# sd196821/QuadSim

Measured on AMD Instinct MI355X. Metric: env-steps/sec at N parallel envs (1/2/4/8 GPU); per-step state L2 err vs NumPy ref, higher is better.
Workload: dtype f32

## Files before the change

### quadsim_amd/csrc/step_kernels.hpp

```cpp
#pragma once

namespace {

#ifndef QS_BLOCK
#define QS_BLOCK 256
#endif
constexpr int kBlock = QS_BLOCK;
#ifndef QS_PREP_MAX_TILES
#define QS_PREP_MAX_TILES 1365
#endif
constexpr int64_t kPrepMaxTiles = QS_PREP_MAX_TILES;
#ifndef QS_SPLIT_MAX_ENVS
#define QS_SPLIT_MAX_ENVS 131072
#endif
constexpr int64_t kSplitMaxEnvs = QS_SPLIT_MAX_ENVS;

struct StepArgs {
    float *st;
    float *par;
    const float *actions;
    float *obs;
    float *reward;
    uint8_t *done;
    uint8_t *flags;
    float *term_obs;
    float *term_state;
    float *slab;
    int64_t n;
    int64_t tile0, tile_end;
    int64_t dbg_shift;
    int64_t io_env0, io_n;
    int64_t T;
    uint64_t step_idx;
    unsigned long long *ctr;
    uint64_t gid0;
    EnvConst C;
    RandCfg rc;
    Par par_nom;
    int auto_reset;
    int randomise;
    float nominal_obs[12];
    const float *init;
    unsigned *owner;
    unsigned *err;
    unsigned long long *stamps;
    unsigned long long stamp_cap, stamp_tiles;
};

__device__ __forceinline__ void load_env(const float *__restrict__ st, int64_t tile, int lane, Env &e)
{
    const float *b = st + tile * (int64_t)(kRecWords * kTile) + lane;
#pragma unroll
    for (int i = 0; i < 13; ++i) e.sc[i] = b[(F_SC + i) * kTile];
#pragma unroll
    for (int i = 0; i < 13; ++i) e.st[i] = b[(F_ST + i) * kTile];
#pragma unroll
    for (int i = 0; i < 4; ++i) e.uc[i] = b[(F_UC + i) * kTile];
#pragma unroll
    for (int i = 0; i < 4; ++i) e.ut[i] = b[(F_UT + i) * kTile];
#pragma unroll
    for (int i = 0; i < 4; ++i) e.qd[i] = b[(F_QD + i) * kTile];
    e.ls = b[F_LS * kTile];
    e.t = b[F_T * kTile];
}

__device__ __forceinline__ void load_env_or_nominal(const StepArgs &A, int64_t tile, int lane, bool active, Env &e)
{
    if (active) load_env(A.st, tile, lane, e);
    else { nominal_init(e.sc, e.st); for (int i = 0; i < 4; ++i) { e.uc[i] = 0.0f; e.ut[i] = 0.0f; e.qd[i] = i == 0; } e.ls = 0.0f; e.t = 0.0f; }
}

__device__ __forceinline__ void store_env(float *__restrict__ st, int64_t tile, int lane, const Env &e)
{
    float *b = st + tile * (int64_t)(kRecWords * kTile) + lane;
#pragma unroll
    for (int i = 0; i < 13; ++i) QS_ST(&b[(F_SC + i) * kTile], e.sc[i]);
#pragma unroll
    for (int i = 0; i < 13; ++i) QS_ST(&b[(F_ST + i) * kTile], e.st[i]);
#pragma unroll
    for (int i = 0; i < 4; ++i) QS_ST(&b[(F_UC + i) * kTile], e.uc[i]);
#pragma unroll
    for (int i = 0; i < 4; ++i) QS_ST(&b[(F_UT + i) * kTile], e.ut[i]);
#pragma unroll
    for (int i = 0; i < 4; ++i) QS_ST(&b[(F_QD + i) * kTile], e.qd[i]);
    QS_ST(&b[F_LS * kTile], e.ls);
    QS_ST(&b[F_T * kTile], e.t);
}

__device__ __forceinline__ Par load_par(const float *__restrict__ par, int64_t tile, int lane)
{
    const float *b = par + tile * (int64_t)(kParWords * kTile) + lane;
    Par P;
    P.m = b[0]; P.Ixx = b[kTile]; P.Iyy = b[2 * kTile]; P.Izz = b[3 * kTile];
    return P;
}

__device__ __forceinline__ void store_par(float *__restrict__ par, int64_t tile, int lane, const Par &P)
{
    float *b = par + tile * (int64_t)(kParWords * kTile) + lane;
    b[0] = P.m; b[kTile] = P.Ixx; b[2 * kTile] = P.Iyy; b[3 * kTile] = P.Izz;
}

struct TileLane { int lane; int64_t tile, env; bool active; };
__device__ __forceinline__ TileLane tile_lane(int64_t n)
{
    const int lane = threadIdx.x & (kTile - 1);
    const int64_t tile = (int64_t)blockIdx.x * (kBlock / kTile) + (threadIdx.x >> 6);
    const int64_t env = tile * kTile + lane;
    return {lane, tile, env, env < n};
}

__device__ __forceinline__ void store_obs(float *__restrict__ obs, int64_t env, const float o[12])
{
    typedef float f4 __attribute__((ext_vector_type(4)));
    f4 *p = reinterpret_cast<f4 *>(obs + env * 12);
    QS_SO(&p[0], (f4{o[0], o[1], o[2], o[3]}));
    QS_SO(&p[1], (f4{o[4], o[5], o[6], o[7]}));
    QS_SO(&p[2], (f4{o[8], o[9], o[10], o[11]}));
}

__device__ __forceinline__ void store_obs_cached(float *__restrict__ obs, int64_t env, const float o[12])
{
    float4 *p = reinterpret_cast<float4 *>(obs + env * 12);
    p[0] = make_float4(o[0], o[1], o[2], o[3]);
    p[1] = make_float4(o[4], o[5], o[6], o[7]);
    p[2] = make_float4(o[8], o[9], o[10], o[11]);
}

__device__ __forceinline__ uint64_t step_counter_begin(const StepArgs &A, int64_t tile) { return A.ctr[tile]; }
__device__ __forceinline__ uint64_t step_counter_begin_vmem(const StepArgs &A, int64_t tile)
{
    int zero;
    asm("v_mov_b32 %0, 0" : "=v"(zero));
    return A.ctr[tile + zero];
}
__device__ __forceinline__ void step_counter_end(const StepArgs &A, int64_t tile, int lane, uint64_t k)
{
    if (lane == 0) A.ctr[tile] = k + (uint64_t)A.T;
}

constexpr unsigned kUnowned = 0xffffffffu;
__device__ __forceinline__ unsigned chain_owner_request(const StepArgs &A, int64_t tile)
{
    const unsigned *p = A.owner ? A.owner + tile : reinterpret_cast<const unsigned *>(A.ctr + tile);
    const unsigned v = __hip_atomic_load(p, __ATOMIC_RELAXED, __HIP_MEMORY_SCOPE_AGENT);
    return A.owner ? v : kUnowned;
}

__device__ __forceinline__ bool chain_owner_mismatch(const StepArgs &A, int64_t tile, int lane, unsigned own)
{
    const unsigned xcc = __builtin_amdgcn_s_getreg((3 << 11) | (0 << 6) | 20) & 15u;
    if (own == kUnowned) {
        unsigned seen = kUnowned;
        if (lane == 0) {
            unsigned expect = kUnowned;
            __hip_atomic_compare_exchange_strong(&A.owner[tile], &expect, xcc, __ATOMIC_RELAXED, __ATOMIC_RELAXED, __HIP_MEMORY_SCOPE_AGENT);
            seen = expect;
        }
        own = __builtin_amdgcn_readfirstlane(seen);
        if (own == kUnowned) return false;
    }
    if (own != xcc) {
        if (lane == 0) __hip_atomic_fetch_or(A.err, 1u, __ATOMIC_RELAXED, __HIP_MEMORY_SCOPE_SYSTEM);
        return true;
    }
    return false;
}

__device__ __forceinline__ bool chain_tile_misplaced(const StepArgs &A, int64_t tile, int lane)
{
    if (!A.owner) return false;
    return chain_owner_mismatch(A, tile, lane, chain_owner_request(A, tile));
}

__device__ __forceinline__ int64_t launch_tile(const StepArgs &A, int64_t b)
{
    const int64_t nt = A.tile_end - A.tile0;
    b += A.dbg_shift;
    b -= (b >= nt) ? nt : 0;
    return A.tile0 + b;
}

template <bool PARAMS, int RMODE>
__device__ __forceinline__ void maybe_reset(Env &e, Par &P, const StepArgs &A, int64_t env, uint64_t k, float obs[12], unsigned flags,
                                            bool &done, bool write_term);

template <int INTEG, bool PARAMS, int RMODE>
__device__ __forceinline__ void step_and_maybe_reset(Env &e, Par &P, const float a[4], const StepArgs &A, int64_t env,
                                                     uint64_t k, float obs[12], float &reward, unsigned &flags,
                                                     bool &done, bool write_term)
{
    env_step<INTEG>(e, a, P, A.C, obs, reward, flags);
    maybe_reset<PARAMS, RMODE>(e, P, A, env, k, obs, flags, done, write_term);
}

template <bool PARAMS, int RMODE>
__device__ __forceinline__ void maybe_reset(Env &e, Par &P, const StepArgs &A, int64_t env, uint64_t k, float obs[12], unsigned flags,
                                            bool &done, bool write_term)
{
    done = (flags & (FLAG_OVERLIMIT | FLAG_OVERTIME)) != 0;
    if (done && A.auto_reset) {
        if (write_term && A.term_obs) store_obs(A.term_obs, env - A.io_env0, obs);
        if (write_term && A.term_state) {
            float *ts = A.term_state + (env - A.io_env0) * 26;
#pragma unroll
            for (int i = 0; i < 13; ++i) { ts[i] = e.sc[i]; ts[13 + i] = e.st[i]; }
        }
        if (RMODE == 0) {
            nominal_init(e.sc, e.st);
#pragma unroll
            for (int i = 0; i < 4; ++i) { e.uc[i] = 0.0f; e.ut[i] = 0.0f; }
            e.ls = 0.0f;
            e.t = 0.0f;
#pragma unroll
            for (int i = 0; i < 12; ++i) obs[i] = A.nominal_obs[i];
        } else if (RMODE == 3) {
            float ic[13], it[13];
            const float *src = A.init + env * 26;
#pragma unroll
            for (int i = 0; i < 13; ++i) { ic[i] = src[i]; it[i] = src[13 + i]; }
            env_reset<false>(e, ic, it, obs);
        } else {
            float ic[13], it[13];
            Par Pn;
            random_init<RMODE == 2>(A.rc, STREAM_AUTORESET, A.gid0 + (uint64_t)env, k + 1, ic, it, Pn);
            if (PARAMS && RMODE == 2) P = Pn;
            env_reset<true>(e, ic, it, obs);
        }
    }
}

template <int INTEG, bool PARAMS, int RMODE>
__global__ __launch_bounds__(kBlock) void k_env(StepArgs A)
{
    const int lane = threadIdx.x & (kTile - 1);
    const int64_t wg_tile = (int64_t)blockIdx.x * (kBlock / kTile) + (threadIdx.x >> 6);
    if (wg_tile >= A.tile_end - A.tile0) return;
    const int64_t tile = launch_tile(A, wg_tile);
    const int64_t env = tile * kTile + lane;
    if (env >= A.n) return;
    if (chain_tile_misplaced(A, tile, lane)) return;
    const int64_t io = env - A.io_env0;
    QS_ASSERT(io >= 0 && io < A.io_n);
    const uint64_t k0 = step_counter_begin_vmem(A, tile);
    float4 av_next = make_float4(0.0f, 0.0f, 0.0f, 0.0f);
    if (A.actions) av_next = reinterpret_cast<const float4 *>(A.actions)[io];
    Env e;
    load_env(A.st, tile, lane, e);
    Par P = A.par_nom;
    if (PARAMS) P = load_par(A.par, tile, lane);
#pragma clang loop unroll(disable)
    for (int64_t t = 0; t < A.T; ++t) {
        const uint64_t k = k0 + (uint64_t)t;
        const int64_t o = t * A.io_n + io;
        float a[4];
        if (A.actions) {
            const float4 av = av_next;
            if (t + 1 < A.T) av_next = reinterpret_cast<const float4 *>(A.actions)[o + A.io_n];
            a[0] = av.x; a[1] = av.y; a[2] = av.z; a[3] = av.w;
        } else {
            random_action(A.rc.seed, A.gid0 + (uint64_t)env, k, a);
        }
        float obs[12], reward;
        unsigned flags;
        bool done;
        step_and_maybe_reset<INTEG, PARAMS, RMODE>(e, P, a, A, env, k, obs, reward, flags, done, true);
        if (A.slab) {
            float2 *row = reinterpret_cast<float2 *>(A.slab + o * 14);
#pragma unroll
            for (int i = 0; i < 6; ++i) row[i] = make_float2(obs[2 * i], obs[2 * i + 1]);
            row[6] = make_float2(reward, done ? 1.0f : 0.0f);
        } else {
            store_obs(A.obs, o, obs);
            QS_SO(&A.reward[o], reward);
            QS_SO(&A.done[o], (uint8_t)(done ? 1 : 0));
        }
        if (A.flags) QS_SO(&A.flags[o], (uint8_t)flags);
    }
    store_env(A.st, tile, lane, e);
    if (PARAMS && RMODE == 2) store_par(A.par, tile, lane, P);
    step_counter_end(A, tile, lane, k0);
}

constexpr int split_waves(int rmode, int prep) { return (prep == 2 && (rmode == 1 || rmode == 2)) ? 3 : 2; }


constexpr bool split_prep(int rmode, int prep) { return split_waves(rmode, prep) == 3; }
constexpr bool split_draw(int rmode, int prep) { return (rmode == 1 || rmode == 2) && !split_prep(rmode, prep); }
template <int RMODE, int PREP>
struct SplitLds {
    float tgt[13][kTile];
    float rst[split_prep(RMODE, PREP) ? 29 : 0][kTile];
    uint4 phx[split_draw(RMODE, PREP) ? 2 : 0][2][kTile];
    unsigned char done[kTile], limt[kTile];
    __device__ __forceinline__ Par reset_par(int lane) const { return Par{rst[25][lane], rst[26][lane], rst[27][lane], rst[28][lane]}; }
};

__device__ __forceinline__ void chaser_load(const float *b, float sc[13], float uc[4], float &ls, float &tt)
{
#pragma unroll
    for (int i = 0; i < 13; ++i) sc[i] = b[(F_SC + i) * kTile];
#pragma unroll
    for (int i = 0; i < 4; ++i) uc[i] = b[(F_UC + i) * kTile];
    ls = b[F_LS * kTile];
    tt = b[F_T * kTile];
}

__device__ __forceinline__ void chaser_store(float *bw, const float sc[13], const float uc[4], float ls, float tt)
{
#pragma unroll
    for (int i = 0; i < 13; ++i) QS_ST(&bw[(F_SC + i) * kTile], sc[i]);
#pragma unroll
    for (int i = 0; i < 4; ++i) QS_ST(&bw[(F_UC + i) * kTile], uc[i]);
    QS_ST(&bw[F_LS * kTile], ls);
    QS_ST(&bw[F_T * kTile], tt);
}

template <int RMODE, int PREP>
__device__ __forceinline__ bool chaser_score(SplitLds<RMODE, PREP> &L, int lane, const float sc[13], const float a[4], float tt, float &ls,
                                             const EnvConst &C, int auto_reset, bool lim_c, float obs[12], float &reward,
                                             unsigned &flags, bool &done)
{
    float st[13];
#pragma unroll
    for (int i = 0; i < 13; ++i) st[i] = L.tgt[i][lane];
    const bool lim_t = L.limt[lane] != 0;
    rel_obs(sc, st, obs);
    score_step(obs, a, sc[2], tt, ls, C, lim_c, lim_t, reward, flags);
    done = (flags & (FLAG_OVERLIMIT | FLAG_OVERTIME)) != 0;
    const bool rs = done && auto_reset;
    L.done[lane] = rs ? 1 : 0;
    return rs;
}

__device__ __forceinline__ void store_term_half(float *term_state, bool active, int64_t io, int half, const float s[13])
{
    if (term_state && active) {
        float *ts = term_state + io * 26 + 13 * half;
#pragma unroll
        for (int i = 0; i < 13; ++i) ts[i] = s[i];
    }
}

template <bool PARAMS, int RMODE, int PREP>
__device__ __forceinline__ void chaser_reset(const SplitLds<RMODE, PREP> &L, const StepArgs &A, int64_t env, bool active, int lane, int64_t t,
                                             float sc[13], float uc[4], float &ls, float &tt, Par &P, float obs[12])
{
    float ic[13], it[13];
    if (RMODE == 0) {
        nominal_init(ic, it);
#pragma unroll
        for (int i = 0; i < 12; ++i) obs[i] = A.nominal_obs[i];
    } else if (RMODE == 3) {
        const float *src = A.init + (active ? env : 0) * 26;
#pragma unroll
        for (int i = 0; i < 13; ++i) { ic[i] = src[i]; it[i] = src[13 + i]; }
        rel_obs<false>(ic, it, obs);
    } else {
        if constexpr (split_prep(RMODE, PREP)) {
#pragma unroll
            for (int i = 0; i < 13; ++i) ic[i] = L.rst[i][lane];
#pragma unroll
            for (int i = 0; i < 12; ++i) obs[i] = L.rst[13 + i][lane];
            if (PARAMS && RMODE == 2) P = L.reset_par(lane);
        } else {
            const uint4 w0 = L.phx[t & 1][0][lane], w1 = RMODE == 2 ? L.phx[t & 1][1][lane] : make_uint4(0, 0, 0, 0);
            Par Pn;
            random_init_apply<RMODE == 2>(A.rc, w0, w1, ic, it, Pn);
            if (PARAMS && RMODE == 2) P = Pn;
            rel_obs<true>(ic, it, obs);
        }
    }
#pragma unroll
    for (int i = 0; i < 13; ++i) sc[i] = ic[i];
#pragma unroll
    for (int i = 0; i < 4; ++i) uc[i] = 0.0f;
    ls = 0.0f;
    tt = 0.0f;
}

__device__ __forceinline__ void target_load(const float *b, float st[13], float ut[4], float qd[4])
{
#pragma unroll
    for (int i = 0; i < 13; ++i) st[i] = b[(F_ST + i) * kTile];
#pragma unroll
    for (int i = 0; i < 4; ++i) ut[i] = b[(F_UT + i) * kTile];
#pragma unroll
    for (int i = 0; i < 4; ++i) qd[i] = b[(F_QD + i) * kTile];
}

__device__ __forceinline__ void target_store(float *bw, const float st[13], const float ut[4], const float qd[4])
{
#pragma unroll
    for (int i = 0; i < 13; ++i) QS_ST(&bw[(F_ST + i) * kTile], st[i]);
#pragma unroll
    for (int i = 0; i < 4; ++i) QS_ST(&bw[(F_UT + i) * kTile], ut[i]);
#pragma unroll
    for (int i = 0; i < 4; ++i) QS_ST(&bw[(F_QD + i) * kTile], qd[i]);
}

template <int RMODE, int PREP>
__device__ __forceinline__ void target_publish(SplitLds<RMODE, PREP> &L, const StepArgs &A, int64_t env, int lane, uint64_t k, int64_t t,
                                               const float st[13], bool lim_t, uint4 &w0, uint4 &w1)
{
#pragma unroll
    for (int i = 0; i < 13; ++i) L.tgt[i][lane] = st[i];
    L.limt[lane] = lim_t ? 1 : 0;
    w0 = make_uint4(0, 0, 0, 0);
    w1 = w0;
    if constexpr (split_draw(RMODE, PREP)) {
        random_init_words<RMODE == 2>(A.rc, STREAM_AUTORESET, A.gid0 + (uint64_t)env, k + 1, w0, w1);
        L.phx[t & 1][0][lane] = w0;
        if (RMODE == 2) L.phx[t & 1][1][lane] = w1;
    }
}

__device__ __forceinline__ void target_command(const EnvConst &C, float qd[4], const float pre[13], float m, float ut[4])
{
    const float pdes[3] = {10.0f, -50.0f, 5.0f};
    const float vdes[3] = {C.vdes_x, 0.0f, 0.0f};
    const float dv[3] = {0.0f, 0.0f, 0.0f};
    float u_t[4];
    target_control(C.kind, pdes, vdes, qd, 0.0f, pre, dv, m, u_t);
    u_limit(u_t, m * kG, ut);
}

template <bool PARAMS, int RMODE, int PREP>
__device__ __forceinline__ void target_reset(const SplitLds<RMODE, PREP> &L, const StepArgs &A, int64_t env, bool active, int lane,
                                             const uint4 &w0, const uint4 &w1, float st[13], float ut[4], Par &P)
{
    float ic[13], it[13];
    if (RMODE == 3) {
        const float *src = A.init + (active ? env : 0) * 26;
#pragma unroll
        for (int i = 0; i < 13; ++i) it[i] = src[13 + i];
    } else {
        nominal_init(ic, it);
        if (PARAMS && RMODE == 2) {
            if constexpr (split_prep(RMODE, PREP)) {
                P = L.reset_par(lane);
            } else {
                random_init_apply<true>(A.rc, w0, w1, ic, it, P);
                nominal_init(ic, it);
            }
        }
    }
#pragma unroll
    for (int i = 0; i < 13; ++i) st[i] = it[i];
#pragma unroll
    for (int i = 0; i < 4; ++i) ut[i] = 0.0f;
}

template <bool PARAMS, int RMODE, int PREP>
__device__ __forceinline__ void prep_publish(SplitLds<RMODE, PREP> &L, const RandCfg &rc, int lane, const uint4 &w0, const uint4 &w1)
{
    float ic[13], it_[13], robs[12];
    Par Pn;
    random_init_apply<RMODE == 2>(rc, w0, w1, ic, it_, Pn);
    rel_obs<true>(ic, it_, robs);
#pragma unroll
    for (int i = 0; i < 13; ++i) L.rst[i][lane] = ic[i];
#pragma unroll
    for (int i = 0; i < 12; ++i) L.rst[13 + i][lane] = robs[i];
    if (PARAMS && RMODE == 2) {
        L.rst[25][lane] = Pn.m; L.rst[26][lane] = Pn.Ixx; L.rst[27][lane] = Pn.Iyy; L.rst[28][lane] = Pn.Izz;
    }
}

constexpr int kResWords = 8;
constexpr unsigned long long kResPtrMask = (1ull << 48) - 1;
enum { RES_STEP = 0, RES_EXIT = 1, RES_IDLE = 2, RES_SKIP = 3 };
constexpr int kResWin = 32;
constexpr int kResWinSlots = 16;

struct ResArgs {
    const unsigned long long *ring;
    unsigned long long *rseq;
    unsigned *wcnt;
    unsigned *fin;
    unsigned long long *h_prog;
    unsigned long long *h_fin;
    unsigned long long seq0;
    unsigned long long base;
    unsigned long long stop_seq;
    unsigned long long slots_mask;
    unsigned long long idle_ticks;
    unsigned lane_tiles;
};

struct ResDesc {
    const float *actions;
    float *obs, *reward;
    uint8_t *done, *flags;
    float *term_obs, *term_state;
};

__device__ __forceinline__ unsigned long long res_request(const ResArgs &R, unsigned long long s, int lane)
{
    return __hip_atomic_load(R.ring + (s & R.slots_mask) * kResWords + (lane & 7), __ATOMIC_RELAXED, __HIP_MEMORY_SCOPE_SYSTEM);
}

__device__ __forceinline__ bool res_fresh(unsigned long long w, unsigned long long s, int lane)
{
    bool ok = (w >> 48) == (s & 0xffffull);
    if ((lane & 7) == 7) ok = ok && (unsigned)w == (unsigned)(s >> 16);
    return __all(ok);
}

__device__ __forceinline__ unsigned long long res_word(unsigned long long w, int i)
{
    const unsigned lo = (unsigned)__builtin_amdgcn_readlane((int)(unsigned)w, i);
    const unsigned hi = (unsigned)__builtin_amdgcn_readlane((int)(unsigned)(w >> 32), i);
    return (((unsigned long long)hi << 32) | lo) & kResPtrMask;
}

__device__ __forceinline__ int res_resolve(const ResArgs &R, unsigned long long s, int lane, unsigned long long w, ResDesc &D)
{
    if (!res_fresh(w, s, lane)) {
        const unsigned long long t0 = __builtin_amdgcn_s_memrealtime();
        for (;;) {
            __builtin_amdgcn_s_sleep(4);
            w = res_request(R, s, lane);
            if (res_fresh(w, s, lane)) break;
            if (__builtin_amdgcn_s_memrealtime() - t0 > R.idle_ticks) return RES_IDLE;
        }
    }
    D.actions = (const float *)res_word(w, 0);
    D.obs = (float *)res_word(w, 1);
    D.reward = (float *)res_word(w, 2);
    D.done = (uint8_t *)res_word(w, 3);
    D.flags = (uint8_t *)res_word(w, 4);
    D.term_obs = (float *)res_word(w, 5);
    D.term_state = (float *)res_word(w, 6);
    return ((res_word(w, 7) >> 32) & 0xff) == 0 ? RES_STEP : RES_EXIT;
}

__device__ __forceinline__ float4 res_action(const float *actions, int64_t io, int64_t io_n)
{
    typedef unsigned u4 __attribute__((ext_vector_type(4)));
    const __amdgpu_buffer_rsrc_t r = __builtin_amdgcn_make_buffer_rsrc((void *)actions, (short)0, (int)(io_n * 16), 0x00020000);
    const u4 v = __builtin_amdgcn_raw_buffer_load_b128(r, (int)(io * 16), 0, 17);
    return make_float4(__uint_as_float(v.x), __uint_as_float(v.y), __uint_as_float(v.z), __uint_as_float(v.w));
}

__device__ __forceinline__ unsigned res_report(const ResArgs &R, unsigned long long s, int64_t tile, int lane)
{
    const unsigned long long x = s - R.base + (unsigned long long)(tile % kResWin) + 1;
    if (x % kResWin != 0) return ~0u;
    unsigned old = 0;
    if (lane == 0) old = __hip_atomic_fetch_add(R.wcnt + (x / kResWin) % kResWinSlots, 1u, __ATOMIC_RELAXED, __HIP_MEMORY_SCOPE_AGENT);
    return old;
}

__device__ __forceinline__ void res_report_done(const ResArgs &R, unsigned old, unsigned long long s, int64_t tile, int lane)
{
    if (old == ~0u || lane != 0 || (old + 1) % R.lane_tiles != 0) return;
    const unsigned long long x = s - R.base + (unsigned long long)(tile % kResWin) + 1;
    __hip_atomic_store(R.h_prog, R.base + x - kResWin + 1, __ATOMIC_RELAXED, __HIP_MEMORY_SCOPE_SYSTEM);
}

template <int INTEG, bool PARAMS, int RMODE, int PREP>
__global__ __launch_bounds__(3 * kTile) void k_env_resident(StepArgs A, ResArgs R)
{
    __shared__ SplitLds<RMODE, PREP> L;
    __shared__ int s_cmd[2];
    __shared__ unsigned long long s_tsp[2];
    const int lane = threadIdx.x & (kTile - 1);
    const int role = threadIdx.x >> 6;
    const int64_t tile = launch_tile(A, blockIdx.x);
    const int64_t env = tile * kTile + lane;
    bool active = env < A.n;
    const int64_t io = env - A.io_env0;
    QS_ASSERT(tile < A.tile_end && (!active || (io >= 0 && io < A.io_n)));
    const uint64_t k0 = step_counter_begin_vmem(A, tile);
    unsigned long long seq = 0;
    int cmd = RES_STEP;
    ResDesc D{};
    {
        if (role == 0) {
            seq = R.seq0 ? R.seq0 : R.rseq[tile];
            seq = ((unsigned long long)__builtin_amdgcn_readfirstlane((int)(unsigned)(seq >> 32)) << 32) |
                  (unsigned)__builtin_amdgcn_readfirstlane((int)(unsigned)seq);
            cmd = seq >= R.stop_seq ? RES_SKIP : res_resolve(R, seq, lane, res_request(R, seq, lane), D);
            if (cmd == RES_STEP) res_report_done(R, res_report(R, seq, tile, lane), seq, tile, lane);
            if (lane == 0) { s_cmd[0] = cmd; s_tsp[0] = (unsigned long long)D.term_state; }
        }
        __syncthreads();
        cmd = s_cmd[0];
    }
    QS_STAMP_DECL;
    QS_STAMP_AT(0);
    const float *b = A.st + tile * (int64_t)(kRecWords * kTile) + lane;
    float *bw = A.st + tile * (int64_t)(kRecWords * kTile) + lane;
    Par P = A.par_nom;
    if (PARAMS) P = load_par(A.par, tile, lane);
    if (role == 0) {
        __builtin_amdgcn_s_setprio(3);
        float sc[13], uc[4], ls, tt;
        chaser_load(b, sc, uc, ls, tt);
        float4 av_next = make_float4(0.0f, 0.0f, 0.0f, 0.0f);
        if (cmd == RES_STEP && active) av_next = res_action(D.actions, io, A.io_n);
#if defined(QS_STAMP) && QS_STAMP + 0 < 2
        asm volatile("s_waitcnt vmcnt(1)" ::: "memory");
#endif
        QS_STAMP_AT(1);
        int64_t t = 0;
#pragma clang loop unroll(disable)
        for (; cmd == RES_STEP; ++t) {
            const int64_t o = io;
            const unsigned long long wn = res_request(R, seq + t + 1, lane);
            tt += 1.0f;
            const bool lim_c = drone_advance<INTEG>(sc, uc, P, A.C.dt);
            float a[4];
            ResDesc Dn{};
            unsigned rep = ~0u;
            const float4 av = av_next;
            const int cmdn = res_resolve(R, seq + t + 1, lane, wn, Dn);
            if (cmdn == RES_STEP) {
                if (active) av_next = res_action(Dn.actions, io, A.io_n);
                rep = res_report(R, seq + t + 1, tile, lane);
            }
            if (lane == 0) { s_cmd[(t + 1) & 1] = cmdn; s_tsp[(t + 1) & 1] = (unsigned long long)Dn.term_state; }
            a[0] = av.x; a[1] = av.y; a[2] = av.z; a[3] = av.w;
            float u_c[4];
            chaser_command(a, P.m, u_c);
            u_limit(u_c, P.m * kG, uc);
            QS_STAMP_AT(2);
            __syncthreads();
            QS_STAMP_AT(3);
            float obs[12], reward;
            unsigned flags;
            bool done;
            const bool rs = chaser_score(L, lane, sc, a, tt, ls, A.C, A.auto_reset, lim_c, obs, reward, flags, done);
            QS_STAMP_AT(4);
            __syncthreads();
            QS_STAMP_AT(5);
            if (rs) {
                if (D.term_obs && active) store_obs(D.term_obs, io, obs);
                store_term_half(D.term_state, active, io, 0, sc);
                chaser_reset<PARAMS>(L, A, env, active, lane, t, sc, uc, ls, tt, P, obs);
            }
            QS_STAMP_AT(6);
            if (active) {
                store_obs(D.obs, o, obs);
                QS_SO(&D.reward[o], reward);
                QS_SO(&D.done[o], (uint8_t)(done ? 1 : 0));
                if (D.flags) QS_SO(&D.flags[o], (uint8_t)flags);
            }
            res_report_done(R, rep, seq + t + 1, tile, lane);
            D = Dn;
            cmd = cmdn;
        }
        if (t > 0) {
            if (active) {
                chaser_store(bw, sc, uc, ls, tt);
                if (PARAMS && RMODE == 2) store_par(A.par, tile, lane, P);
            }
        }
        {
            if (cmd != RES_SKIP && lane == 0) {
                if (t > 0) A.ctr[tile] = k0 + (uint64_t)t;
                R.rseq[tile] = seq + (unsigned long long)t + (cmd == RES_EXIT ? 1 : 0);
                if (cmd == RES_EXIT) {
                    const unsigned old = __hip_atomic_fetch_add(R.fin, 1u, __ATOMIC_RELAXED, __HIP_MEMORY_SCOPE_AGENT);
                    if (old + 1 == R.lane_tiles)
                        __hip_atomic_store(R.h_fin, seq + (unsigned long long)t + 1, __ATOMIC_RELAXED, __HIP_MEMORY_SCOPE_SYSTEM);
                }
            }
        }
#if defined(QS_STAMP) && QS_STAMP + 0 < 2
        asm volatile("s_waitcnt vmcnt(0)" ::: "memory");
#endif
        QS_STAMP_AT(7);
        QS_STAMP_FLUSH();
    } else if (role == 1) {
        float st[13], ut[4], qd[4];
        target_load(b, st, ut, qd);
#if defined(QS_STAMP) && QS_STAMP + 0 < 2
        asm volatile("s_waitcnt vmcnt(0)" ::: "memory");
#endif
        QS_STAMP_AT(1);
        int64_t t = 0;
#pragma clang loop unroll(disable)
        for (; cmd == RES_STEP; ++t) {
            float pre[13];
#pragma unroll
            for (int i = 0; i < 13; ++i) pre[i] = st[i];
            const bool lim_t = drone_advance<INTEG>(st, ut, P, A.C.dt);
            uint4 w0, w1;
            target_publish(L, A, env, lane, k0 + (uint64_t)t, t, st, lim_t, w0, w1);
            QS_STAMP_AT(2);
            __syncthreads();
            QS_STAMP_AT(3);
            float *const term_state = (float *)s_tsp[t & 1];
            target_command(A.C, qd, pre, P.m, ut);
            QS_STAMP_AT(4);
            __syncthreads();
            QS_STAMP_AT(5);
            if (L.done[lane]) {
                store_term_half(term_state, active, io, 1, st);
                target_reset<PARAMS>(L, A, env, active, lane, w0, w1, st, ut, P);
            }
            cmd = s_cmd[(t + 1) & 1];
        }
        if (active && t > 0) target_store(bw, st, ut, qd);
        QS_STAMP_AT(6);
        QS_STAMP_FLUSH();
    } else if constexpr (split_prep(RMODE, PREP)) {
        int64_t t = 0;
#pragma clang loop unroll(disable)
        for (; cmd == RES_STEP; ++t) {
            uint4 w0, w1 = make_uint4(0, 0, 0, 0);
            random_init_words<RMODE == 2>(A.rc, STREAM_AUTORESET, A.gid0 + (uint64_t)env, k0 + (uint64_t)t + 1, w0, w1);
            __syncthreads();
            prep_publish<PARAMS>(L, A.rc, lane, w0, w1);
            __syncthreads();
            cmd = s_cmd[(t + 1) & 1];
        }
    }
}

template <int INTEG, bool PARAMS, int RMODE, int PREP>
__global__ __launch_bounds__(3 * kTile) void k_env_split(StepArgs A)
{
    __shared__ SplitLds<RMODE, PREP> L;
    const int lane = threadIdx.x & (kTile - 1);
    const int role = threadIdx.x >> 6;
    const int64_t tile = launch_tile(A, blockIdx.x);
    const int64_t env = tile * kTile + lane;
    bool active = env < A.n;
    const int64_t io = env - A.io_env0;
    QS_ASSERT(tile < A.tile_end && (!active || (io >= 0 && io < A.io_n)));
    const unsigned owner_xcc = chain_owner_request(A, tile);
    const uint64_t k0 = step_counter_begin_vmem(A, tile);
    QS_STAMP_DECL;
    QS_STAMP_AT(0);
    const float *b = A.st + tile * (int64_t)(kRecWords * kTile) + lane;
    float *bw = A.st + tile * (int64_t)(kRecWords * kTile) + lane;
    Par P = A.par_nom;
    if (PARAMS) P = load_par(A.par, tile, lane);
    if (role == 0) {
        if (A.T > 1) __builtin_amdgcn_s_setprio(3);
        float sc[13], uc[4], ls, tt;
        chaser_load(b, sc, uc, ls, tt);
        float4 av_next = make_float4(0.0f, 0.0f, 0.0f, 0.0f);
        if (A.actions && active) av_next = reinterpret_cast<const float4 *>(A.actions)[io];
#if defined(QS_STAMP) && QS_STAMP + 0 < 2
        asm volatile("s_waitcnt vmcnt(1)" ::: "memory");
#endif
        QS_STAMP_AT(1);
#pragma clang loop unroll(disable)
        for (int64_t t = 0; t < A.T; ++t) {
            const uint64_t k = k0 + (uint64_t)t;
            const int64_t o = t * A.io_n + io;
            tt += 1.0f;
            const bool lim_c = drone_advance<INTEG>(sc, uc, P, A.C.dt);
            if (A.owner && chain_owner_mismatch(A, tile, lane, owner_xcc)) active = false;
            float a[4];
            if (A.actions) {
                const float4 av = av_next;
                if (t + 1 < A.T && active) av_next = reinterpret_cast<const float4 *>(A.actions)[o + A.io_n];
                a[0] = av.x; a[1] = av.y; a[2] = av.z; a[3] = av.w;
            } else {
                random_action(A.rc.seed, A.gid0 + (uint64_t)env, k, a);
            }
            float u_c[4];
            chaser_command(a, P.m, u_c);
            u_limit(u_c, P.m * kG, uc);
            QS_STAMP_AT(2);
            __syncthreads();
            QS_STAMP_AT(3);
            if (A.T == 1) __builtin_amdgcn_s_setprio(3);
            float obs[12], reward;
            unsigned flags;
            bool done;
            const bool rs = chaser_score(L, lane, sc, a, tt, ls, A.C, A.auto_reset, lim_c, obs, reward, flags, done);
            QS_STAMP_AT(4);
            __syncthreads();
            QS_STAMP_AT(5);
            if (rs) {
                if (A.term_obs && active) store_obs(A.term_obs, io, obs);
                store_term_half(A.term_state, active, io, 0, sc);
                chaser_reset<PARAMS>(L, A, env, active, lane, t, sc, uc, ls, tt, P, obs);
            }
            QS_STAMP_AT(6);
            if (active) {
                if (A.slab) {
                    float2 *row = reinterpret_cast<float2 *>(A.slab + o * 14);
#pragma unroll
                    for (int i = 0; i < 6; ++i) row[i] = make_float2(obs[2 * i], obs[2 * i + 1]);
                    row[6] = make_float2(reward, done ? 1.0f : 0.0f);
                } else {
                    store_obs(A.obs, o, obs);
                    QS_SO(&A.reward[o], reward);
                    QS_SO(&A.done[o], (uint8_t)(done ? 1 : 0));
                }
                if (A.flags) QS_SO(&A.flags[o], (uint8_t)flags);
            }
        }
        if (active) {
            chaser_store(bw, sc, uc, ls, tt);
            if (PARAMS && RMODE == 2) store_par(A.par, tile, lane, P);
        }
        if (!A.owner || active || env >= A.n) step_counter_end(A, tile, lane, k0);
#if defined(QS_STAMP) && QS_STAMP + 0 < 2
        asm volatile("s_waitcnt vmcnt(0)" ::: "memory");
#endif
        QS_STAMP_AT(7);
        QS_STAMP_FLUSH();
    } else if (role == 1) {
        float st[13], ut[4], qd[4];
        target_load(b, st, ut, qd);
        if (A.T == 1) __builtin_amdgcn_s_setprio(3);
#if defined(QS_STAMP) && QS_STAMP + 0 < 2
        asm volatile("s_waitcnt vmcnt(0)" ::: "memory");
#endif
        QS_STAMP_AT(1);
#pragma clang loop unroll(disable)
        for (int64_t t = 0; t < A.T; ++t) {
            float pre[13];
#pragma unroll
            for (int i = 0; i < 13; ++i) pre[i] = st[i];
            const bool lim_t = drone_advance<INTEG>(st, ut, P, A.C.dt);
            if (A.owner && chain_owner_mismatch(A, tile, lane, owner_xcc)) active = false;
            uint4 w0, w1;
            target_publish(L, A, env, lane, k0 + (uint64_t)t, t, st, lim_t, w0, w1);
            QS_STAMP_AT(2);
            __syncthreads();
            QS_STAMP_AT(3);
            if (A.T == 1) __builtin_amdgcn_s_setprio(0);
            target_command(A.C, qd, pre, P.m, ut);
            QS_STAMP_AT(4);
            __syncthreads();
            QS_STAMP_AT(5);
            if (L.done[lane]) {
                store_term_half(A.term_state, active, io, 1, st);
                target_reset<PARAMS>(L, A, env, active, lane, w0, w1, st, ut, P);
            }
        }
        if (active) target_store(bw, st, ut, qd);
        QS_STAMP_AT(6);
        QS_STAMP_FLUSH();
    } else if constexpr (split_prep(RMODE, PREP)) {
#pragma clang loop unroll(disable)
        for (int64_t t = 0; t < A.T; ++t) {
            uint4 w0, w1 = make_uint4(0, 0, 0, 0);
            random_init_words<RMODE == 2>(A.rc, STREAM_AUTORESET, A.gid0 + (uint64_t)env, k0 + (uint64_t)t + 1, w0, w1);
            __syncthreads();
            prep_publish<PARAMS>(L, A.rc, lane, w0, w1);
            __syncthreads();
        }
    }
}

template <int INTEG, bool PARAMS>
__global__ __launch_bounds__(kBlock) void k_hover(StepArgs A)
{
    const int lane = threadIdx.x & (kTile - 1);
    const int64_t tile = A.tile0 + (int64_t)blockIdx.x * (kBlock / kTile) + (threadIdx.x >> 6);
    const int64_t env = tile * kTile + lane;
    if (tile >= A.tile_end || env >= A.n) return;
    const int64_t io = env - A.io_env0;
    QS_ASSERT(io >= 0 && io < A.io_n);
    const uint64_t k0 = step_counter_begin(A, tile);
    float *b = A.st + tile * (int64_t)(kRecWords * kTile) + lane;
    float s[13], up[4];
#pragma unroll
    for (int i = 0; i < 13; ++i) s[i] = b[(F_SC + i) * kTile];
#pragma unroll
    for (int i = 0; i < 4; ++i) up[i] = b[(F_UC + i) * kTile];
    Par P = A.par_nom;
    if (PARAMS) P = load_par(A.par, tile, lane);
#pragma clang loop unroll(disable)
    for (int64_t t = 0; t < A.T; ++t) {
        const int64_t o = t * A.io_n + io;
        float a[4];
        if (A.actions) {
            const float4 av = reinterpret_cast<const float4 *>(A.actions)[o];
            a[0] = av.x; a[1] = av.y; a[2] = av.z; a[3] = av.w;
        } else {
            random_action(A.rc.seed, A.gid0 + (uint64_t)env, k0 + (uint64_t)t, a);
#pragma unroll
            for (int i = 0; i < 4; ++i) a[i] = 0.5f * a[i] + 0.5f;
        }
        float reward;
        unsigned flags;
        hover_step<INTEG>(s, up, a, P, A.C.dt, reward, flags);
        const bool done = (flags & FLAG_OVERLIMIT) != 0;
        if (done && A.auto_reset) {
            if (A.term_obs) for (int i = 0; i < 13; ++i) A.term_obs[io * 13 + i] = s[i];
            const float *src = A.init + env * 13;
#pragma unroll
            for (int i = 0; i < 13; ++i) s[i] = src[i];
#pragma unroll
            for (int i = 0; i < 4; ++i) up[i] = 0.0f;
        }
#pragma unroll
        for (int i = 0; i < 13; ++i) A.obs[o * 13 + i] = s[i];
        A.reward[o] = reward;
        A.done[o] = done ? 1 : 0;
        if (A.flags) A.flags[o] = (uint8_t)flags;
    }
#pragma unroll
    for (int i = 0; i < 13; ++i) b[(F_SC + i) * kTile] = s[i];
#pragma unroll
    for (int i = 0; i < 4; ++i) b[(F_UC + i) * kTile] = up[i];
    step_counter_end(A, tile, lane, k0);
}

__global__ __launch_bounds__(kBlock) void k_ctor_init(float *init, int64_t n, int hover, uint64_t seed, uint64_t gid0)
{
    const int64_t env = (int64_t)blockIdx.x * kBlock + threadIdx.x;
    if (env >= n) return;
    uint4 w = philox_block(seed, STREAM_CTOR, gid0 + (uint64_t)env, 0);
    if (!hover) {
        float *d = init + env * 26;
        for (int i = 0; i < 26; ++i) d[i] = 0.0f;
        d[0] = __fmaf_rn(sym(u16lo(w.x)), 0.3f, 8.0f);
        d[1] = __fmaf_rn(sym(u16hi(w.x)), 0.3f, -50.0f);
        d[2] = __fmaf_rn(sym(u16lo(w.y)), 0.3f, 5.0f);
        d[6] = 1.0f;
        d[13] = 10.0f; d[14] = -50.0f; d[15] = 5.0f; d[19] = 1.0f;
    } else {
        float *d = init + env * 13;
        for (int i = 0; i < 13; ++i) d[i] = 0.0f;
        d[0] = sym(u16lo(w.x));
        d[1] = sym(u16hi(w.x));
        d[2] = __fmaf_rn(sym(u16lo(w.y)), 1.0f, 5.0f);
        float e0 = sym(u16hi(w.y)) * 0.2f, e1 = sym(u16lo(w.z)) * 0.2f, e2 = sym(u16hi(w.z)) * 0.2f;
        float sr, cr, sp, cp, sy, cy;
        q_sincos_small(0.5f * e0, sr, cr);
        q_sincos_small(0.5f * e1, sp, cp);
        q_sincos_small(0.5f * e2, sy, cy);
        euler2quat_trig(sr, cr, sp, cp, sy, cy, d + 6);
    }
}

__global__ __launch_bounds__(kBlock) void k_fill_init_nominal(float *init, int64_t n)
{
    const int64_t env = (int64_t)blockIdx.x * kBlock + threadIdx.x;
    if (env >= n) return;
    float sc[13], st[13];
    nominal_init(sc, st);
    for (int i = 0; i < 13; ++i) { init[env * 26 + i] = sc[i]; init[env * 26 + 13 + i] = st[i]; }
}

__global__ __launch_bounds__(kBlock) void k_reset(StepArgs A, const uint8_t *__restrict__ mask, int init_all)
{
    const int lane = threadIdx.x & (kTile - 1);
    const int64_t tile = (int64_t)blockIdx.x * (kBlock / kTile) + (threadIdx.x >> 6);
    const int64_t env = tile * kTile + lane;
    if (env >= A.n) return;
    if (mask && !mask[env]) return;
    Env e;
    load_env(A.st, tile, lane, e);
    float ic[13], it[13], obs[12];
    if (A.init) {
        const float *src = A.init + env * 26;
        for (int i = 0; i < 13; ++i) { ic[i] = src[i]; it[i] = src[13 + i]; }
    } else if (A.randomise) {
        Par Pn;
        random_init<true>(A.rc, STREAM_RESET, A.gid0 + (uint64_t)env, A.ctr[tile], ic, it, Pn);
        if (A.randomise >= 2) store_par(A.par, tile, lane, Pn);
    } else {
        nominal_init(ic, it);
    }
    if (init_all) { e.qd[0] = 1.0f; e.qd[1] = 0.0f; e.qd[2] = 0.0f; e.qd[3] = 0.0f; }
    env_reset(e, ic, it, obs);
    store_env(A.st, tile, lane, e);
    if (A.obs) store_obs(A.obs, env, obs);
}

__global__ __launch_bounds__(kBlock) void k_hover_reset(StepArgs A, const uint8_t *__restrict__ mask)
{
    const int lane = threadIdx.x & (kTile - 1);
    const int64_t tile = (int64_t)blockIdx.x * (kBlock / kTile) + (threadIdx.x >> 6);
    const int64_t env = tile * kTile + lane;
    if (env >= A.n) return;
    if (mask && !mask[env]) return;
    float *b = A.st + tile * (int64_t)(kRecWords * kTile) + lane;
    const float *src = A.init + env * 13;
    for (int i = 0; i < 13; ++i) { b[(F_SC + i) * kTile] = src[i]; if (A.obs) A.obs[env * 13 + i] = src[i]; }
    for (int i = 0; i < 4; ++i) b[(F_UC + i) * kTile] = 0.0f;
}

__global__ __launch_bounds__(kBlock) void k_fill_ctr(unsigned long long *ctr, int64_t tiles, unsigned long long k)
{
    const int64_t i = (int64_t)blockIdx.x * kBlock + threadIdx.x;
    if (i < tiles) ctr[i] = k;
}

__global__ void k_nominal_obs(float *out)
{
    float sc[13], st[13], o[12];
    nominal_init(sc, st);
    rel_obs(sc, st, o);
    for (int i = 0; i < 12; ++i) out[i] = o[i];
}

__global__ __launch_bounds__(kBlock) void k_fill_par(float *par, int64_t n, Par P)
{
    const int lane = threadIdx.x & (kTile - 1);
    const int64_t tile = (int64_t)blockIdx.x * (kBlock / kTile) + (threadIdx.x >> 6);
    if (tile * kTile + lane >= n) return;
    store_par(par, tile, lane, P);
}

__global__ __launch_bounds__(kBlock) void k_fill_actions(float *__restrict__ actions, int64_t n, int64_t T, uint64_t seed,
                                                         uint64_t gid0, uint64_t step0)
{
    const int64_t i = (int64_t)blockIdx.x * kBlock + threadIdx.x;
    if (i >= n * T) return;
    const int64_t t = i / n, env = i - t * n;
    float a[4];
    random_action(seed, gid0 + (uint64_t)env, step0 + (uint64_t)t, a);
    reinterpret_cast<float4 *>(actions)[i] = make_float4(a[0], a[1], a[2], a[3]);
}

struct StateIO {
    float *chaser, *target, *u_prev, *qdes, *ls, *t;
};
template <bool TO_USER>
__global__ __launch_bounds__(kBlock) void k_state_io(float *st, int64_t n, StateIO io)
{
    const int lane = threadIdx.x & (kTile - 1);
    const int64_t tile = (int64_t)blockIdx.x * (kBlock / kTile) + (threadIdx.x >> 6);
    const int64_t env = tile * kTile + lane;
    if (env >= n) return;
    float *b = st + tile * (int64_t)(kRecWords * kTile) + lane;
    auto mv = [&](float *user, int f) {
        if (!user) return;
        if (TO_USER) *user = b[f * kTile];
        else b[f * kTile] = *user;
    };
    for (int i = 0; i < 13; ++i) mv(io.chaser ? io.chaser + env * 13 + i : nullptr, F_SC + i);
    for (int i = 0; i < 13; ++i) mv(io.target ? io.target + env * 13 + i : nullptr, F_ST + i);
    for (int i = 0; i < 8; ++i) mv(io.u_prev ? io.u_prev + env * 8 + i : nullptr, F_UC + i);
    for (int i = 0; i < 4; ++i) mv(io.qdes ? io.qdes + env * 4 + i : nullptr, F_QD + i);
    mv(io.ls ? io.ls + env : nullptr, F_LS);
    mv(io.t ? io.t + env : nullptr, F_T);
}

template <bool TO_USER>
__global__ __launch_bounds__(kBlock) void k_par_io(float *par, int64_t n, float *mass, float *inertia)
{
    const int lane = threadIdx.x & (kTile - 1);
    const int64_t tile = (int64_t)blockIdx.x * (kBlock / kTile) + (threadIdx.x >> 6);
    const int64_t env = tile * kTile + lane;
    if (env >= n) return;
    float *b = par + tile * (int64_t)(kParWords * kTile) + lane;
    if (TO_USER) {
        if (mass) mass[env] = b[0];
        if (inertia) for (int i = 0; i < 3; ++i) inertia[env * 3 + i] = b[(1 + i) * kTile];
    } else {
        if (mass) b[0] = mass[env];
        if (inertia) for (int i = 0; i < 3; ++i) b[(1 + i) * kTile] = inertia[env * 3 + i];
    }
}

inline int64_t tiles_of(int64_t n) { return (n + kTile - 1) / kTile; }
inline unsigned grid_tiles(int64_t n) { return (unsigned)((tiles_of(n) + (kBlock / kTile) - 1) / (kBlock / kTile)); }
inline unsigned grid_flat(int64_t n) { return (unsigned)((n + kBlock - 1) / kBlock); }

}
```

Baseline: 26.28 billion.

## Move resident-loop progress reporting off the chaser wave to the last wave

Moves the per-step window progress atomics (res_report/res_report_done) from the critical chaser wave onto the last wave of the block (target or prep), passing the sequence number through LDS. Casts descriptor pointers to the global address space so the compiler emits global rather than flat memory ops, and pins the prefetched action values with an inline-asm move so the next action load can be issued earlier. The intent is to shorten the chaser wave's per-step critical path, at the cost of extra cross-wave coordination and an unconditional waitcnt before the loop.

```diff
diff --git a/quadsim_amd/csrc/step_kernels.hpp b/quadsim_amd/csrc/step_kernels.hpp
--- a/quadsim_amd/csrc/step_kernels.hpp
+++ b/quadsim_amd/csrc/step_kernels.hpp
@@ -507,6 +507,12 @@
     return __all(ok);
 }
 
+template <typename T>
+__device__ __forceinline__ T *res_ptr(unsigned long long a)
+{
+    return (T *)(__attribute__((address_space(1))) T *)a;
+}
+
 __device__ __forceinline__ unsigned long long res_word(unsigned long long w, int i)
 {
     const unsigned lo = (unsigned)__builtin_amdgcn_readlane((int)(unsigned)w, i);
@@ -525,13 +531,13 @@
             if (__builtin_amdgcn_s_memrealtime() - t0 > R.idle_ticks) return RES_IDLE;
         }
     }
-    D.actions = (const float *)res_word(w, 0);
-    D.obs = (float *)res_word(w, 1);
-    D.reward = (float *)res_word(w, 2);
-    D.done = (uint8_t *)res_word(w, 3);
-    D.flags = (uint8_t *)res_word(w, 4);
-    D.term_obs = (float *)res_word(w, 5);
-    D.term_state = (float *)res_word(w, 6);
+    D.actions = res_ptr<const float>(res_word(w, 0));
+    D.obs = res_ptr<float>(res_word(w, 1));
+    D.reward = res_ptr<float>(res_word(w, 2));
+    D.done = res_ptr<uint8_t>(res_word(w, 3));
+    D.flags = res_ptr<uint8_t>(res_word(w, 4));
+    D.term_obs = res_ptr<float>(res_word(w, 5));
+    D.term_state = res_ptr<float>(res_word(w, 6));
     return ((res_word(w, 7) >> 32) & 0xff) == 0 ? RES_STEP : RES_EXIT;
 }
 
@@ -541,6 +547,13 @@
     const __amdgpu_buffer_rsrc_t r = __builtin_amdgcn_make_buffer_rsrc((void *)actions, (short)0, (int)(io_n * 16), 0x00020000);
     const u4 v = __builtin_amdgcn_raw_buffer_load_b128(r, (int)(io * 16), 0, 17);
     return make_float4(__uint_as_float(v.x), __uint_as_float(v.y), __uint_as_float(v.z), __uint_as_float(v.w));
+}
+
+__device__ __forceinline__ float res_keep(float v)
+{
+    float r;
+    asm volatile("v_mov_b32 %0, %1" : "=v"(r) : "v"(v));
+    return r;
 }
 
 __device__ __forceinline__ unsigned res_report(const ResArgs &R, unsigned long long s, int64_t tile, int lane)
@@ -559,12 +572,15 @@
     __hip_atomic_store(R.h_prog, R.base + x - kResWin + 1, __ATOMIC_RELAXED, __HIP_MEMORY_SCOPE_SYSTEM);
 }
 
+constexpr int res_reporter(int rmode, int prep) { return split_waves(rmode, prep) - 1; }
 template <int INTEG, bool PARAMS, int RMODE, int PREP>
 __global__ __launch_bounds__(3 * kTile) void k_env_resident(StepArgs A, ResArgs R)
 {
     __shared__ SplitLds<RMODE, PREP> L;
     __shared__ int s_cmd[2];
     __shared__ unsigned long long s_tsp[2];
+    __shared__ unsigned long long s_seq;
+    constexpr int kRep = res_reporter(RMODE, PREP);
     const int lane = threadIdx.x & (kTile - 1);
     const int role = threadIdx.x >> 6;
     const int64_t tile = launch_tile(A, blockIdx.x);
@@ -583,10 +599,15 @@
                   (unsigned)__builtin_amdgcn_readfirstlane((int)(unsigned)seq);
             cmd = seq >= R.stop_seq ? RES_SKIP : res_resolve(R, seq, lane, res_request(R, seq, lane), D);
             if (cmd == RES_STEP) res_report_done(R, res_report(R, seq, tile, lane), seq, tile, lane);
-            if (lane == 0) { s_cmd[0] = cmd; s_tsp[0] = (unsigned long long)D.term_state; }
+            if (lane == 0) { s_cmd[0] = cmd; s_tsp[0] = (unsigned long long)D.term_state; s_seq = seq; }
         }
         __syncthreads();
         cmd = s_cmd[0];
+        if (role == kRep) {
+            seq = s_seq;
+            seq = ((unsigned long long)__builtin_amdgcn_readfirstlane((int)(unsigned)(seq >> 32)) << 32) |
+                  (unsigned)__builtin_amdgcn_readfirstlane((int)(unsigned)seq);
+        }
     }
     QS_STAMP_DECL;
     QS_STAMP_AT(0);
@@ -604,6 +625,7 @@
         asm volatile("s_waitcnt vmcnt(1)" ::: "memory");
 #endif
         QS_STAMP_AT(1);
+        __builtin_amdgcn_s_waitcnt(0x0f70);
         int64_t t = 0;
 #pragma clang loop unroll(disable)
         for (; cmd == RES_STEP; ++t) {
@@ -613,15 +635,10 @@
             const bool lim_c = drone_advance<INTEG>(sc, uc, P, A.C.dt);
             float a[4];
             ResDesc Dn{};
-            unsigned rep = ~0u;
-            const float4 av = av_next;
             const int cmdn = res_resolve(R, seq + t + 1, lane, wn, Dn);
-            if (cmdn == RES_STEP) {
-                if (active) av_next = res_action(Dn.actions, io, A.io_n);
-                rep = res_report(R, seq + t + 1, tile, lane);
-            }
+            a[0] = res_keep(av_next.x); a[1] = res_keep(av_next.y); a[2] = res_keep(av_next.z); a[3] = res_keep(av_next.w);
+            if (cmdn == RES_STEP && active) av_next = res_action(Dn.actions, io, A.io_n);
             if (lane == 0) { s_cmd[(t + 1) & 1] = cmdn; s_tsp[(t + 1) & 1] = (unsigned long long)Dn.term_state; }
-            a[0] = av.x; a[1] = av.y; a[2] = av.z; a[3] = av.w;
             float u_c[4];
             chaser_command(a, P.m, u_c);
             u_limit(u_c, P.m * kG, uc);
@@ -647,7 +664,6 @@
                 QS_SO(&D.done[o], (uint8_t)(done ? 1 : 0));
                 if (D.flags) QS_SO(&D.flags[o], (uint8_t)flags);
             }
-            res_report_done(R, rep, seq + t + 1, tile, lane);
             D = Dn;
             cmd = cmdn;
         }
@@ -692,7 +708,10 @@
             QS_STAMP_AT(2);
             __syncthreads();
             QS_STAMP_AT(3);
-            float *const term_state = (float *)s_tsp[t & 1];
+            float *const term_state = res_ptr<float>(s_tsp[t & 1]);
+            const int cmdn = s_cmd[(t + 1) & 1];
+            unsigned rep = ~0u;
+            if (kRep == 1 && cmdn == RES_STEP) rep = res_report(R, seq + t + 1, tile, lane);
             target_command(A.C, qd, pre, P.m, ut);
             QS_STAMP_AT(4);
             __syncthreads();
@@ -701,7 +720,8 @@
                 store_term_half(term_state, active, io, 1, st);
                 target_reset<PARAMS>(L, A, env, active, lane, w0, w1, st, ut, P);
             }
-            cmd = s_cmd[(t + 1) & 1];
+            if (kRep == 1) res_report_done(R, rep, seq + t + 1, tile, lane);
+            cmd = cmdn;
         }
         if (active && t > 0) target_store(bw, st, ut, qd);
         QS_STAMP_AT(6);
@@ -713,9 +733,12 @@
             uint4 w0, w1 = make_uint4(0, 0, 0, 0);
             random_init_words<RMODE == 2>(A.rc, STREAM_AUTORESET, A.gid0 + (uint64_t)env, k0 + (uint64_t)t + 1, w0, w1);
             __syncthreads();
+            const int cmdn = s_cmd[(t + 1) & 1];
+            const unsigned rep = cmdn == RES_STEP ? res_report(R, seq + t + 1, tile, lane) : ~0u;
             prep_publish<PARAMS>(L, A.rc, lane, w0, w1);
             __syncthreads();
-            cmd = s_cmd[(t + 1) & 1];
+            res_report_done(R, rep, seq + t + 1, tile, lane);
+            cmd = cmdn;
         }
     }
 }
```

After: 25.66 billion. 2.4% lower.
